# cybera/distributed_tensorflow_ibm_mnist

Measured on AMD Instinct MI355X. Metric: images/sec (whole node) MNIST LeNet-5, higher is better.
Workload: dtype bf16; 1 GPU; model=LeNet-5, global_batch=65536, per_gpu_batch=65536, parallelism=dp1, impl=hip, hip_graph=False, optimizer=momentum, input=bf16, input_lookahead=True

## Files before the change

### csrc/kernels/lenet_bwd.hip

```cpp
#include <cstdlib>
#include <cstring>

#include "common.h"
#include "launchers.h"
#include "wgrad_tr.h"

namespace mnistx {
namespace {


constexpr int NT = 1024, NW = 16, T = 8;
constexpr int NWIN1 = 196;
constexpr int AF_OFF = 0, AF_SZ = 15 * 64 * 16;
constexpr int DY2_RS = 384, DY2_IMG = 3872;
constexpr int DY2_OFF = AF_OFF + AF_SZ, DY2_SZ = T * DY2_IMG;
constexpr int ZERO_OFF = DY2_OFF + DY2_SZ;
constexpr int P1_RS = 272, P1_IMG = 3808;
constexpr int P1_OFF = ZERO_OFF + DY2_RS, P1_SZ = T * P1_IMG;
constexpr int X_RS = 80, X_IMG = 2592;
constexpr int X_OFF = P1_OFF + P1_SZ, X_SZ = T * X_IMG;
constexpr int D_RS = 280, D_IMG = 3920;
constexpr int DP1_OFF = X_OFF + X_SZ, D_SZ = T * D_IMG;
constexpr int CD_OFF = DP1_OFF + D_SZ;
constexpr int LDS_BYTES = CD_OFF + D_SZ;
static_assert(LDS_BYTES <= 163840, "one workgroup per CU");
static_assert(10 * DY2_RS <= DY2_IMG && 32 * X_RS <= X_IMG && 14 * P1_RS <= P1_IMG && 14 * D_RS <= D_IMG, "");
static_assert((ZERO_OFF - DY2_OFF) % 256 == 0, "zero row bank-aligned with the dY2 rows (bench/lds_bwd.py)");
constexpr int C2MAX = 4;
static_assert(NW * C2MAX * 256 * 4 <= LDS_BYTES && NW * 6 * 256 * 4 + NW * 8 * 4 <= LDS_BYTES, "epilogue scratch");

constexpr int C2_TAP0[13] = {0, 2, 5, 7, 10, 12, 15, 17, 20, 22, 4, 14, 24};
constexpr int C2_GT[4][C2MAX] = {{0, 1, 2, 3}, {4, 5, 10, -1}, {6, 7, 11, -1}, {8, 9, 12, -1}};
__constant__ int c2_gt[4][C2MAX] = {{0, 1, 2, 3}, {4, 5, 10, -1}, {6, 7, 11, -1}, {8, 9, 12, -1}};
__constant__ int c2_tap0[13] = {0, 2, 5, 7, 10, 12, 15, 17, 20, 22, 4, 14, 24};

struct BwdArgs {
  const bf16_t* x;
  const uint8_t* u8;
  const int64_t* idx;
  int n;
  const bf16_t* p1;
  const bf16_t* dp2;
  const uint8_t* arg2;
  const bf16_t* w2;
  int B;
  float* slab1;
  float* slab2;
  unsigned long long* prof;
  int skip;
  int prof_waves;
  int8_t du[16], k20[16], k21[16], k10[8], k11[8];
};
constexpr int NPROF = 8;

constexpr int NCH = 2;
static_assert(NW == 2 * T && 2 * 128 >= NWIN1 && 128 <= NWIN1, "staging: one wave pair per image, 2 chunks");
template <bool U8, bool IDX>
struct Stage {
  u32x2 x[NCH];
  u32x2 rowv;
  u32x4 dp;
  u32x2 c2;
  u32x4 p1[NCH];

  DEV static int img_of(int wave) { return wave >> 1; }
  DEV void load_row(const BwdArgs& a, int t0, int wave) {
    if constexpr (IDX) {
      const int img = img_of(wave);
      const bool ok = t0 >= 0 && t0 + img < a.B;
      const auto ridx = buf_rsrc(a.idx + (ok ? t0 + img : 0), ok ? 8u : 0u);
      rowv = buf_b64(ridx, 0u);
    }
  }
  DEV void load_xc(const BwdArgs& a, int t0, int wave, int ln) {
    const int img = img_of(wave);
    const bool ok = t0 >= 0 && t0 + img < a.B;
    int row = ok ? t0 + img : 0;
    if constexpr (IDX) {
      const uint32_t lo = __builtin_amdgcn_readfirstlane(rowv[0]), hi = __builtin_amdgcn_readfirstlane(rowv[1]);
      row = (hi != 0u || (int)lo < 0) ? 0 : ((int)lo >= a.n ? a.n - 1 : (int)lo);
    }
    constexpr uint32_t esz = U8 ? 1u : 2u;
    const void* xb = U8 ? (const void*)(a.u8 + (int64_t)row * 784) : (const void*)(a.x + (int64_t)row * 784);
    const auto rx = buf_rsrc(xb, ok ? 784u * esz : 0u);
    const int r = ln + 64 * (wave & 1);
#pragma unroll
    for (int i = 0; i < NCH; ++i) {
      const uint32_t q = (uint32_t)(r + 128 * i);
      const uint32_t oob = q < NWIN1 ? 0u : BUF_OOB;
      if constexpr (U8) x[i] = u32x2{buf_b32(rx, 4u * q + oob), 0u};
      else x[i] = buf_b64(rx, 8u * q + oob);
    }
  }
  DEV void store_xc(uint8_t* lds, int wave, int ln) const {
    const int img = img_of(wave), r = ln + 64 * (wave & 1);
#pragma unroll
    for (int i = 0; i < NCH; ++i) {
      const int q = r + 128 * i;
      if (i == 0 || q < NWIN1) {
        const int y = (q * 147) >> 10, k = q - 7 * y;
        const int yp = (q * 147) >> 11, xp = q - 14 * yp;
        uint32_t lo = x[i][0], hi = x[i][1];
        if constexpr (U8) {
          const uint32_t b = x[i][0];
          lo = pack2(u8_norm(b & 0xff), u8_norm((b >> 8) & 0xff));
          hi = pack2(u8_norm((b >> 16) & 0xff), u8_norm(b >> 24));
        }
        *(u32x2*)(lds + X_OFF + img * X_IMG + (y + 2) * X_RS + (4 * k + 4) * 2) = u32x2{lo, hi};
        const uint32_t a1 = p1[i][3];
        const uint32_t l4 = a1 & 0x0f0f0f0fu, h4 = (a1 >> 4) & 0x0f0f0f0fu;
        uint8_t* cd = lds + CD_OFF + img * D_IMG + yp * D_RS + xp * 16;
        *(u32x2*)cd = u32x2{bytes01(l4), bytes23(l4)};
        *(u32x2*)(cd + 8) = u32x2{bytes01(h4), bytes23(h4)};
      }
    }
  }
  DEV void load_dy(const BwdArgs& a, int t0, int wave, int ln) {
    const int nimg = t0 < 0 ? 0 : min(T, a.B - t0);
    const int tb = t0 < 0 ? 0 : t0;
    const int tid = wave * 64 + ln;
    const auto rdp = buf_rsrc(a.dp2 + (int64_t)tb * 400, (uint32_t)nimg * 800u);
    const auto ra2 = buf_rsrc(a.arg2 + (int64_t)tb * 400, (uint32_t)nimg * 400u);
    dp = buf_b128(rdp, tid < 400 ? 16u * tid : BUF_OOB);
    c2 = buf_b64(ra2, tid < 400 ? 8u * tid : BUF_OOB);
    const int img = img_of(wave);
    const bool ok = t0 >= 0 && t0 + img < a.B;
    const auto rp1 = buf_rsrc(a.p1 + (int64_t)(ok ? t0 + img : 0) * NWIN1 * 8, ok ? NWIN1 * 16u : 0u);
    const int r = ln + 64 * (wave & 1);
#pragma unroll
    for (int i = 0; i < NCH; ++i) {
      const uint32_t q = (uint32_t)(r + 128 * i);
      p1[i] = a.skip & 32 ? u32x4{0u, 0u, 0u, 0u} : buf_b128(rp1, q < NWIN1 ? 16u * q : BUF_OOB);
    }
  }
  DEV void store_dy(uint8_t* lds, int wave, int ln) {
    asm volatile("" : "+v"(dp), "+v"(c2), "+v"(p1[0]), "+v"(p1[1]));
    const int img = img_of(wave), r = ln + 64 * (wave & 1);
#pragma unroll
    for (int i = 0; i < NCH; ++i) {
      const int q = r + 128 * i;
      if (i == 0 || q < NWIN1) {
        const int yp = (q * 147) >> 11, xp = q - 14 * yp;
        const u32x4 v = {p1[i][0], p1[i][1], p1[i][2], 0x3f80u};
        *(u32x4*)(lds + P1_OFF + img * P1_IMG + yp * P1_RS + xp * 16) = v;
      }
    }
    const int tid = wave * 64 + ln;
    if (tid < 400) {
      const int im = tid / 50, rr = tid - 50 * im, w = rr >> 1, yp = w / 5, xp = w - 5 * yp;
      const int o = DY2_OFF + im * DY2_IMG + 2 * yp * DY2_RS + 2 * xp * 32 + 16 * (rr & 1);
      const uint32_t e[4] = {bytes01(c2[0]), bytes23(c2[0]), bytes01(c2[1]), bytes23(c2[1])};
      const int rot = (xp >> 1) & 1;
#pragma unroll
      for (int i = 0; i < 4; ++i) {
        const int d = i ^ rot;
        const uint32_t dd = (uint32_t)d * 0x00010001u;
        const u32x4 v = {sel_eq(dp[0], e[0], dd), sel_eq(dp[1], e[1], dd), sel_eq(dp[2], e[2], dd),
                         sel_eq(dp[3], e[3], dd)};
        *(u32x4*)(lds + o + (i >> 1) * DY2_RS + (d & 1) * 32) = v;
      }
    }
  }
};

template <int H>
DEV void dgrad_unit(const uint8_t* lds, int bB, int bZ, int orow, int lane, int dylo, int dyhi, f32x4 (&acc)[4]) {
  constexpr int VLO = H ? 2 : 0, VHI = H ? 4 : 3, NU = H ? 3 : 4;
#pragma unroll 2
  for (int dy = dylo; dy <= dyhi; ++dy) {
    bf16x8 Bv[VHI - VLO + 1];
    const int r = orow - dy;
    const uint8_t* pb = lds + ((unsigned)r <= 9u ? bB - dy * DY2_RS : bZ);
#pragma unroll
    for (int v = VLO; v <= VHI; ++v) Bv[v - VLO] = *(const bf16x8*)(pb + 64 * v);
#pragma unroll
    for (int j = 0; j < 3; ++j) {
      const bf16x8 A = *(const bf16x8*)(lds + AF_OFF + ((dy * 3 + j) * 64 + lane) * 16);
#pragma unroll
      for (int v = VLO; v <= VHI; ++v) {
        const int u = v + 2 - j - 4 * H;
        if (u >= 0 && u < NU) acc[u] = mfma16(A, Bv[v - VLO], acc[u]);
      }
    }
  }
}

template <int G>
DEV void c2w_steps(const uint8_t* lds, int ks0, int ks1, int ln, f32x4 (&acc2)[C2MAX]) {
  const int g = ln >> 4, q = (ln >> 2) & 3, p = ln & 3;
  const int img = 4 * (g & 1) + q, sub = 2 * (g >> 1), hA = p >> 1, pc = p & 1;
  const int bB = DY2_OFF + img * DY2_IMG + sub * 32 + 8 * p;
  const int aB = P1_OFF + img * P1_IMG + sub * 16 + 8 * pc;
  const int aP = aB + hA * 16, aR = aB + hA * P1_RS;
  constexpr int NT2 = G == 0 ? 4 : 3;
#pragma unroll 2
  for (int s = ks0; s < ks1; ++s) {
    const int y = s / 3, x0 = 4 * (s - 3 * y);
    const int sb = bB + y * DY2_RS + x0 * 32, sa = y * P1_RS + x0 * 16;
    const bf16x8 Bf = frag(tr4(lds, sb), tr4(lds, sb + 32));
#pragma unroll
    for (int t = 0; t < NT2; ++t) {
      const int tile = C2_GT[G][t], tap = C2_TAP0[tile];
      const int base = (tile < 10 ? aP : aR) + sa + (tap / 5) * P1_RS + (tap % 5) * 16;
      acc2[t] = mfma16(frag(tr4(lds, base), tr4(lds, base + 16)), Bf, acc2[t]);
    }
  }
}

constexpr int8_t DG_UNIT[NW] = {7, 5, 9, 4, 6, 10, 3, 8, 2, 11, 0, 1, 12, 13, -1, -1};
constexpr int8_t C2_KS0[NW] = {0, 6, 13, 23, 0, 8, 16, 23, 0, 7, 15, 22, 0, 7, 14, 22};
constexpr int8_t C2_KS1[NW] = {6, 13, 23, 30, 8, 16, 23, 30, 7, 15, 22, 30, 7, 14, 22, 30};
constexpr int8_t C1_KS0[8] = {0, 4, 8, 12, 16, 20, 24, 26};
constexpr int8_t C1_KS1[8] = {4, 8, 12, 16, 20, 24, 26, 28};

template <bool PROF, bool U8, bool IDX>
__global__ __launch_bounds__(NT, 1) void lenet_bwd_k(const BwdArgs a) {
  extern __shared__ __attribute__((aligned(16))) uint8_t lds[];
  const int tid = threadIdx.x, lane = tid & 63, wave = __builtin_amdgcn_readfirstlane(tid >> 6);
  const int ntiles = (a.B + T - 1) / T;
  const int nk = ntiles > (int)blockIdx.x ? (ntiles - 1 - (int)blockIdx.x) / (int)gridDim.x + 1 : 0;
  auto tile0 = [&](int k) { return k < nk ? ((int)blockIdx.x + k * (int)gridDim.x) * T : -1; };

  for (int e = tid; e < LDS_BYTES / 16; e += NT) *(u32x4*)(lds + 16 * e) = u32x4{0u, 0u, 0u, 0u};
  __syncthreads();
  if (tid < 15 * 64) {
    const int f = tid >> 6, dy = f / 3, j = f - 3 * dy;
    const int r = (lane & 15) >> 3, ci = lane & 7, xs = lane >> 5, co0 = 8 * ((lane >> 4) & 1);
    const int dx = r + 4 - 2 * j - xs;
    u32x4 v = {0u, 0u, 0u, 0u};
    if (dx >= 0 && dx <= 4) v = *(const u32x4*)(a.w2 + ((dy * 5 + dx) * 8 + ci) * 16 + co0);
    *(u32x4*)(lds + AF_OFF + 16 * tid) = v;
  }
  Stage<U8, IDX> st;
  st.load_row(a, tile0(0), wave);
  st.load_xc(a, tile0(0), wave, lane);
  st.load_dy(a, tile0(0), wave, lane);
  st.load_row(a, tile0(1), wave);
  st.store_dy(lds, wave, lane);

  const int grp = wave >> 2, sig = wave & 1;
  f32x4 acc2[C2MAX];
#pragma unroll
  for (int t = 0; t < C2MAX; ++t) acc2[t] = f32x4{0.f, 0.f, 0.f, 0.f};
  f32x4 acc1[3][2];
#pragma unroll
  for (int t = 0; t < 3; ++t) acc1[t][0] = acc1[t][1] = f32x4{0.f, 0.f, 0.f, 0.f};
  float db1[4] = {0.f, 0.f, 0.f, 0.f};
  const int du = a.du[wave];
  const int ks0 = a.k20[wave], ks1 = a.k21[wave];
  const int cs0 = a.k10[wave >> 1], cs1 = a.k11[wave >> 1];

  uint64_t pc_acc[NPROF] = {0, 0, 0, 0, 0, 0, 0, 0};
  uint64_t tclk = __builtin_amdgcn_s_memtime();
  auto mark = [&](int ph) {
    if constexpr (PROF) {
      const uint64_t t = __builtin_amdgcn_s_memtime();
      pc_acc[ph] += t - tclk;
      tclk = t;
    }
  };

  for (int k = 0; k < nk; ++k) {
    const int t0 = tile0(k);
    if (!(PROF && (a.skip & 16))) __syncthreads();
    mark(6);
    if (!(PROF && (a.skip & 8))) {
      const int ln = lane_now();
      st.store_xc(lds, wave, ln);
    }
    mark(0);

    if (du >= 0 && !(PROF && (a.skip & 1))) {
      const int ln = lane_now();
      const int i16 = ln & 15, g = ln >> 4;
      const int pr = du >> 1, hx = du & 1;
      const int img = i16 >> 1, rr = i16 & 1, orow = 2 * pr + rr;
      const int dylo = max(0, 2 * pr - 9), dyhi = min(4, 2 * pr + 1);
      const int u0 = 4 * hx;
      u32x2 pv[4];
#pragma unroll
      for (int u = 0; u < 4; ++u)
        pv[u] = *(const u32x2*)(lds + P1_OFF + img * P1_IMG + orow * P1_RS + (2 * min(u0 + u, 6) + (g >> 1)) * 16 +
                                8 * (g & 1));
      if (!(PROF && (a.skip & 8))) st.load_xc(a, tile0(k + 1), wave, ln);
      f32x4 acc[4];
#pragma unroll
      for (int u = 0; u < 4; ++u) acc[u] = f32x4{0.f, 0.f, 0.f, 0.f};
      const int lo = (g >> 1) * 32 + (g & 1) * 16;
      const int bB = DY2_OFF + img * DY2_IMG + orow * DY2_RS + lo, bZ = ZERO_OFF + lo;
      if (hx) dgrad_unit<1>(lds, bB, bZ, orow, ln, dylo, dyhi, acc);
      else dgrad_unit<0>(lds, bB, bZ, orow, ln, dylo, dyhi, acc);
      const int wB = DP1_OFF + img * D_IMG + orow * D_RS + (2 * u0 + (g >> 1)) * 16 + 8 * (g & 1);
#pragma unroll
      for (int u = 0; u < 4; ++u) {
        if (u0 + u < 7) {
          *(u32x2*)(lds + wB + 32 * u) = u32x2{pack2(acc[u][0], acc[u][1]), pack2(acc[u][2], acc[u][3])};
#pragma unroll
          for (int i = 0; i < 4; ++i) {
            const int16_t pvi = (int16_t)((pv[u][i >> 1] >> (16 * (i & 1))) & 0xffffu);
            db1[i] = fmaf(acc[u][i], pvi > 0 ? 1.f : 0.f, db1[i]);
          }
        }
      }
    } else if (!(PROF && (a.skip & 8))) {
      st.load_xc(a, tile0(k + 1), wave, lane_now());
    }
    if (!(PROF && (a.skip & 8))) st.load_dy(a, tile0(k + 1), wave, lane_now());
    mark(1);

    if (ks0 < ks1 && !(PROF && (a.skip & 2))) {
      const int ln = lane_now();
      switch (grp) {
        case 0: c2w_steps<0>(lds, ks0, ks1, ln, acc2); break;
        case 1: c2w_steps<1>(lds, ks0, ks1, ln, acc2); break;
        case 2: c2w_steps<2>(lds, ks0, ks1, ln, acc2); break;
        default: c2w_steps<3>(lds, ks0, ks1, ln, acc2); break;
      }
    }

    mark(2);
    if (!(PROF && (a.skip & 16))) __syncthreads();
    mark(3);
    if (!(PROF && (a.skip & 8))) st.load_row(a, tile0(k + 2), wave);
    mark(4);

    {
      const int ln = lane_now(), g = ln >> 4, q = (ln >> 2) & 3, p = ln & 3;
      const int img = 4 * (g & 1) + q, sub = 2 * (g >> 1), hA = p >> 1, pc = p & 1;
      const uint32_t dsel = (uint32_t)((ln & 15) >> 3);
      const uint32_t dd0 = dsel * 0x00010001u, dd1 = (2u + dsel) * 0x00010001u;
      const int aB = X_OFF + img * X_IMG + hA * X_RS + (4 * sub + 4 * pc + 4 * sig) * 2;
      const int bB = DP1_OFF + img * D_IMG + (2 * sub + sig) * 16 + 8 * pc;
#pragma unroll 2
      for (int s = cs0; s < (PROF && (a.skip & 4) ? cs0 : cs1); ++s) {
        const int yp = s >> 1, xi0 = 4 * (s & 1);
        const int sa = aB + 2 * yp * X_RS + 8 * xi0, sb = bB + yp * D_RS + 32 * xi0;
        const u32x4 dv = __builtin_bit_cast(u32x4, frag(tr4(lds, sb), tr4(lds, sb + 32)));
        const u32x4 cv = __builtin_bit_cast(u32x4, frag(tr4(lds, sb + (CD_OFF - DP1_OFF)),
                                                         tr4(lds, sb + (CD_OFF - DP1_OFF) + 32)));
        const bf16x8 B0 = __builtin_bit_cast(bf16x8, u32x4{sel_eq(dv[0], cv[0], dd0), sel_eq(dv[1], cv[1], dd0),
                                                           sel_eq(dv[2], cv[2], dd0), sel_eq(dv[3], cv[3], dd0)});
        const bf16x8 B1 = __builtin_bit_cast(bf16x8, u32x4{sel_eq(dv[0], cv[0], dd1), sel_eq(dv[1], cv[1], dd1),
                                                           sel_eq(dv[2], cv[2], dd1), sel_eq(dv[3], cv[3], dd1)});
#pragma unroll
        for (int t = 0; t < 3; ++t) {
          const bf16x8 Af = frag(tr4(lds, sa + 2 * t * X_RS), tr4(lds, sa + 2 * t * X_RS + 8));
          acc1[t][0] = mfma16(Af, B0, acc1[t][0]);
          acc1[t][1] = mfma16(Af, B1, acc1[t][1]);
        }
      }
    }
    if (k + 1 < nk && !(PROF && (a.skip & 8))) st.store_dy(lds, wave, lane_now());
    mark(5);
  }

  const int i16 = lane & 15, g = lane >> 4;
  __syncthreads();
  mark(6);
  float* e2 = (float*)lds;
#pragma unroll
  for (int t = 0; t < C2MAX; ++t) *(f32x4*)(e2 + ((wave * C2MAX + t) * 16 + i16) * 16 + 4 * g) = acc2[t];
  __syncthreads();
  float* s2 = a.slab2 + (int64_t)blockIdx.x * 208 * 16;
  for (int e = tid; e < 4 * C2MAX * 256; e += NT) {
    const int G = e >> 10, t = (e >> 8) & 3, row = (e >> 4) & 15, col = e & 15;
    const int tile = c2_gt[G][t];
    if (tile < 0) continue;
    const int h = row >> 3, ci = row & 7, tap = c2_tap0[tile] + h * (tile < 10 ? 1 : 5);
    const bool bias = tile == 0 && h == 0 && ci == 6;
    if (tap >= 25 || (ci >= 6 && !bias)) continue;
    float v = 0.f;
#pragma unroll
    for (int w = 0; w < 4; ++w) v += e2[(((4 * G + w) * C2MAX + t) * 16 + col) * 16 + row];
    s2[(bias ? 200 : tap * 8 + ci) * 16 + col] = v;
  }
  __syncthreads();
  float* e1 = (float*)lds;
#pragma unroll
  for (int t = 0; t < 3; ++t)
#pragma unroll
    for (int nt = 0; nt < 2; ++nt)
      *(f32x4*)(e1 + (((wave * 3 + t) * 2 + nt) * 16 + i16) * 16 + 4 * g) = acc1[t][nt];
#pragma unroll
  for (int i = 0; i < 4; ++i) {
#pragma unroll
    for (int m = 1; m <= 32; m = m == 8 ? 32 : 2 * m) db1[i] += __shfl_xor(db1[i], m);
  }
  float* eb = e1 + NW * 6 * 256;
  if (lane == 0 || lane == 16) *(f32x4*)(eb + wave * 8 + (lane >> 2)) = f32x4{db1[0], db1[1], db1[2], db1[3]};
  __syncthreads();
  float* s1 = a.slab1 + (int64_t)blockIdx.x * 32 * 8;
  if (tid < 26 * 8) {
    const int tap = tid >> 3, c = tid & 7;
    float v = 0.f;
    if (tap < 25) {
      const int dy = tap / 5, dx = tap - 5 * dy;
      for (int w = 0; w < NW; ++w) {
        const int s = w & 1;
#pragma unroll
        for (int d = 0; d < 4; ++d) {
          const int ty = dy + (d >> 1), tx = dx + (d & 1), txi = tx + (s ? 0 : 2);
          const int t = ty >> 1, row = 4 * (2 * (ty & 1) + (txi >> 2)) + (txi & 3);
          const int nt = d >> 1, col = c + 8 * (d & 1);
          v += e1[(((w * 3 + t) * 2 + nt) * 16 + col) * 16 + row];
        }
      }
    } else {
      for (int w = 0; w < NW; ++w) v += eb[w * 8 + c];
    }
    s1[tap * 8 + c] = v;
  }
  if constexpr (PROF) {
    mark(7);
    __syncthreads();
    unsigned long long* ep = (unsigned long long*)lds;
    if (lane == 0)
      for (int i = 0; i < NPROF; ++i) ep[wave * NPROF + i] = pc_acc[i];
    __syncthreads();
    if (tid < NPROF) {
      unsigned long long v = 0;
      for (int w = 0; w < NW; ++w) v += ep[w * NPROF + tid];
      atomicAdd(a.prof + tid, v);
    }
    if (a.prof_waves && tid < NW * NPROF) atomicAdd(a.prof + NPROF + tid, ep[tid]);
  }
}

struct BwdSplit {
  int8_t du[16], k20[16], k21[16], k10[8], k11[8];
  bool ok;
};
BwdSplit bwd_split() {
  BwdSplit s{};
  memcpy(s.du, DG_UNIT, 16);
  memcpy(s.k20, C2_KS0, 16);
  memcpy(s.k21, C2_KS1, 16);
  memcpy(s.k10, C1_KS0, 8);
  memcpy(s.k11, C1_KS1, 8);
  s.ok = true;
  const char* e = getenv("MNISTX_BWD_SPLIT");
  if (!e || !*e) return s;
  int v[64], n = 0;
  for (const char* p = e; *p && n < 64;) {
    char* end = nullptr;
    const long x = strtol(p, &end, 10);
    if (end == p) break;
    v[n++] = (int)x;
    p = *end == ',' ? end + 1 : end;
  }
  if (n != 64) return BwdSplit{{}, {}, {}, {}, {}, false};
  int seen[14] = {};
  for (int w = 0; w < 16; ++w) {
    if (v[w] < -1 || v[w] > 13) return BwdSplit{{}, {}, {}, {}, {}, false};
    if (v[w] >= 0) ++seen[v[w]];
  }
  for (int u = 0; u < 14; ++u)
    if (seen[u] != 1) return BwdSplit{{}, {}, {}, {}, {}, false};
  for (int G = 0; G < 4; ++G) {
    int cover[30] = {};
    for (int t = 0; t < 4; ++t) {
      const int w = 4 * G + t, k0 = v[16 + w], k1 = v[32 + w];
      if (k0 < 0 || k1 < k0 || k1 > 30) return BwdSplit{{}, {}, {}, {}, {}, false};
      for (int k = k0; k < k1; ++k) ++cover[k];
    }
    for (int k = 0; k < 30; ++k)
      if (cover[k] != 1) return BwdSplit{{}, {}, {}, {}, {}, false};
  }
  int cover1[28] = {};
  for (int r = 0; r < 8; ++r) {
    const int k0 = v[48 + r], k1 = v[56 + r];
    if (k0 < 0 || k1 < k0 || k1 > 28) return BwdSplit{{}, {}, {}, {}, {}, false};
    for (int k = k0; k < k1; ++k) ++cover1[k];
  }
  for (int k = 0; k < 28; ++k)
    if (cover1[k] != 1) return BwdSplit{{}, {}, {}, {}, {}, false};
  for (int i = 0; i < 16; ++i) {
    s.du[i] = (int8_t)v[i];
    s.k20[i] = (int8_t)v[16 + i];
    s.k21[i] = (int8_t)v[32 + i];
  }
  for (int i = 0; i < 8; ++i) {
    s.k10[i] = (int8_t)v[48 + i];
    s.k11[i] = (int8_t)v[56 + i];
  }
  return s;
}

using BwdKernel = void (*)(BwdArgs);
constexpr BwdKernel kBwd[8] = {lenet_bwd_k<false, false, false>, lenet_bwd_k<false, false, true>,
                               lenet_bwd_k<false, true, false>,  lenet_bwd_k<false, true, true>,
                               lenet_bwd_k<true, false, false>,  lenet_bwd_k<true, false, true>,
                               lenet_bwd_k<true, true, false>,   lenet_bwd_k<true, true, true>};

}

int lenet_bwd_grid(int* per_cu = nullptr) {
  static int n = 0, per = 0;
  if (n == 0) {
    int dev = 0, cus = 0;
    for (BwdKernel k : kBwd)
      if (hipFuncSetAttribute((const void*)k, hipFuncAttributeMaxDynamicSharedMemorySize, LDS_BYTES) != hipSuccess)
        return -1;
    if (hipOccupancyMaxActiveBlocksPerMultiprocessor(&per, kBwd[0], NT, LDS_BYTES) != hipSuccess ||
        hipGetDevice(&dev) != hipSuccess ||
        hipDeviceGetAttribute(&cus, hipDeviceAttributeMultiprocessorCount, dev) != hipSuccess || per <= 0)
      return -1;
    n = per * cus;
  }
  if (per_cu) *per_cu = per;
  return n;
}

hipError_t lenet_bwd(const XSrc& x, const bf16_t* p1, const bf16_t* dp2, const uint8_t* arg2, const bf16_t* w2,
                     int B, float* slab1, float* slab2, int grid, hipStream_t st, unsigned long long* prof) {
  if (B <= 0) return hipSuccess;
  if ((!x.x && !x.u8) || grid <= 0) return hipErrorInvalidValue;
  const int res = lenet_bwd_grid();
  if (res <= 0) return hipErrorInvalidValue;
  BwdArgs a{x.u8 ? nullptr : x.x, x.u8, x.idx, x.idx ? x.n : B, p1, dp2, arg2, w2, B, slab1, slab2, prof, 0, 0,
            {}, {}, {}, {}, {}};
  static const BwdSplit sp = bwd_split();
  if (!sp.ok) return hipErrorInvalidValue;
  memcpy(a.du, sp.du, 16);
  memcpy(a.k20, sp.k20, 16);
  memcpy(a.k21, sp.k21, 16);
  memcpy(a.k10, sp.k10, 8);
  memcpy(a.k11, sp.k11, 8);
  if (prof) {
    const char* e = getenv("MNISTX_BWD_SKIP");
    a.skip = e ? atoi(e) : 0;
    const char* pw = getenv("MNISTX_BWD_PROF_WAVES");
    a.prof_waves = (pw && pw[0] == '1') ? 1 : 0;
  }
  const BwdKernel k = kBwd[(prof ? 4 : 0) + (x.u8 ? 2 : 0) + (x.idx ? 1 : 0)];
  void* args[] = {&a};
  return hipLaunchKernel((const void*)k, dim3(grid), dim3(NT), args, LDS_BYTES, st);
}

int lenet_bwd_blocks(int B) {
  int per = 1;
  const int full = lenet_bwd_grid(&per);
  if (full <= 0) return -1;
  const int res = reserve_cut(full, per);
  const int ntiles = (B + T - 1) / T;
  return cap_grid(ntiles < res ? ntiles : res);
}

}
```

Baseline: 168.8 million images/s.

## Software-pipeline LDS loads against MFMAs in backward dgrad and wgrad loops

Adds pipelined versions of the conv2 dgrad, conv2 wgrad and conv1 wgrad inner loops. Each loop prefetches the next step's A/B fragments from LDS while the current step's MFMAs issue, and uses sched_barrier to keep that interleaving fixed. The goal is to hide LDS latency behind matrix-core work, at the cost of more live registers and a fixed instruction schedule. The pipelined kernel is the default and can be turned off with the MNISTX_BWD_PIPE=0 environment variable.

```diff
diff --git a/csrc/kernels/lenet_bwd.hip b/csrc/kernels/lenet_bwd.hip
--- a/csrc/kernels/lenet_bwd.hip
+++ b/csrc/kernels/lenet_bwd.hip
@@ -9,6 +9,9 @@
 namespace {
 
 
+#ifndef BWD_PIPE_LOOPS
+#define BWD_PIPE_LOOPS 7
+#endif
 constexpr int NT = 1024, NW = 16, T = 8;
 constexpr int NWIN1 = 196;
 constexpr int AF_OFF = 0, AF_SZ = 15 * 64 * 16;
@@ -115,6 +118,11 @@
       }
     }
   }
+  DEV void drop_xc() { x[0] = x[1] = u32x2{0u, 0u}; }
+  DEV void drop_dy() {
+    dp = p1[0] = p1[1] = u32x4{0u, 0u, 0u, 0u};
+    c2 = u32x2{0u, 0u};
+  }
   DEV void load_dy(const BwdArgs& a, int t0, int wave, int ln) {
     const int nimg = t0 < 0 ? 0 : min(T, a.B - t0);
     const int tb = t0 < 0 ? 0 : t0;
@@ -182,6 +190,53 @@
         if (u >= 0 && u < NU) acc[u] = mfma16(A, Bv[v - VLO], acc[u]);
       }
     }
+  }
+}
+
+constexpr int8_t DG_J[2][9] = {{0, 1, 2, 0, 1, 2, 1, 2, 2}, {0, 0, 0, 1, 1, 2, -1, -1, -1}};
+constexpr int8_t DG_V[2][9] = {{0, 0, 0, 1, 1, 1, 2, 2, 3}, {2, 3, 4, 3, 4, 4, -1, -1, -1}};
+constexpr bool dg_last_j(int H, int n) {
+  for (int m = n + 1; m < 9; ++m)
+    if (DG_J[H][m] == DG_J[H][n]) return false;
+  return true;
+}
+constexpr bool dg_last_v(int H, int n) {
+  for (int m = n + 1; m < 9; ++m)
+    if (DG_V[H][m] == DG_V[H][n]) return false;
+  return true;
+}
+template <int H>
+DEV void dgrad_unit_pipe(const uint8_t* lds, int bB, int bZ, int orow, int lane, int dylo, int dyhi,
+                         f32x4 (&acc)[4]) {
+  constexpr int VLO = H ? 2 : 0, VHI = H ? 4 : 3, NM = H ? 6 : 9;
+  auto rowp = [&](int dy) {
+    const int r = orow - dy;
+    return lds + ((unsigned)r <= 9u ? bB - dy * DY2_RS : bZ);
+  };
+  auto ldA = [&](int dy, int j) { return *(const bf16x8*)(lds + AF_OFF + ((dy * 3 + j) * 64 + lane) * 16); };
+  bf16x8 Bv[VHI - VLO + 1], A[3];
+  {
+    const uint8_t* pb = rowp(dylo);
+#pragma unroll
+    for (int v = VLO; v <= VHI; ++v) Bv[v - VLO] = *(const bf16x8*)(pb + 64 * v);
+#pragma unroll
+    for (int j = 0; j < 3; ++j) A[j] = ldA(dylo, j);
+  }
+  for (int dy = dylo; dy < dyhi; ++dy) {
+    const uint8_t* pn = rowp(dy + 1);
+#pragma unroll
+    for (int n = 0; n < NM; ++n) {
+      const int j = DG_J[H][n], v = DG_V[H][n], u = v + 2 - j - 4 * H;
+      acc[u] = mfma16(A[j], Bv[v - VLO], acc[u]);
+      __builtin_amdgcn_sched_barrier(0);
+      if (dg_last_j(H, n)) A[j] = ldA(dy + 1, j);
+      if (dg_last_v(H, n)) Bv[v - VLO] = *(const bf16x8*)(pn + 64 * v);
+    }
+  }
+#pragma unroll
+  for (int n = 0; n < NM; ++n) {
+    const int j = DG_J[H][n], v = DG_V[H][n], u = v + 2 - j - 4 * H;
+    acc[u] = mfma16(A[j], Bv[v - VLO], acc[u]);
   }
 }
 
@@ -207,13 +262,124 @@
   }
 }
 
+template <int G>
+DEV void c2w_steps_pipe(const uint8_t* lds, int ks0, int ks1, int ln, f32x4 (&acc2)[C2MAX]) {
+  if (ks0 >= ks1) return;
+  const int g = ln >> 4, q = (ln >> 2) & 3, p = ln & 3;
+  const int img = 4 * (g & 1) + q, sub = 2 * (g >> 1), hA = p >> 1, pc = p & 1;
+  const int bB = DY2_OFF + img * DY2_IMG + sub * 32 + 8 * p;
+  const int aB = P1_OFF + img * P1_IMG + sub * 16 + 8 * pc;
+  const int aP = aB + hA * 16, aR = aB + hA * P1_RS;
+  constexpr int NT2 = G == 0 ? 4 : 3;
+  auto ldB = [&](int s) {
+    const int y = s / 3, x0 = 4 * (s - 3 * y);
+    const int sb = bB + y * DY2_RS + x0 * 32;
+    return frag(tr4(lds, sb), tr4(lds, sb + 32));
+  };
+  auto ldA = [&](int s, int t) {
+    const int y = s / 3, x0 = 4 * (s - 3 * y);
+    const int tile = C2_GT[G][t], tap = C2_TAP0[tile];
+    const int base = (tile < 10 ? aP : aR) + y * P1_RS + x0 * 16 + (tap / 5) * P1_RS + (tap % 5) * 16;
+    return frag(tr4(lds, base), tr4(lds, base + 16));
+  };
+  bf16x8 A[NT2], Ba = ldB(ks0), Bb;
+#pragma unroll
+  for (int t = 0; t < NT2; ++t) A[t] = ldA(ks0, t);
+  auto step = [&](int sn, const bf16x8& Bc, bf16x8& Bn) {
+    Bn = ldB(sn);
+#pragma unroll
+    for (int t = 0; t < NT2; ++t) {
+      acc2[t] = mfma16(A[t], Bc, acc2[t]);
+      __builtin_amdgcn_sched_barrier(0);
+      A[t] = ldA(sn, t);
+    }
+  };
+  auto drain = [&](const bf16x8& Bc) {
+#pragma unroll
+    for (int t = 0; t < NT2; ++t) acc2[t] = mfma16(A[t], Bc, acc2[t]);
+  };
+  int sn = ks0 + 1;
+  for (; sn + 1 < ks1; sn += 2) {
+    step(sn, Ba, Bb);
+    step(sn + 1, Bb, Ba);
+  }
+  if (sn < ks1) {
+    step(sn, Ba, Bb);
+    drain(Bb);
+  } else {
+    drain(Ba);
+  }
+}
+
+DEV void c1w_steps_pipe(const uint8_t* lds, int cs0, int cs1, int ln, int sig, f32x4 (&acc1)[3][2]) {
+  if (cs0 >= cs1) return;
+  const int g = ln >> 4, q = (ln >> 2) & 3, p = ln & 3;
+  const int img = 4 * (g & 1) + q, sub = 2 * (g >> 1), hA = p >> 1, pc = p & 1;
+  const uint32_t dsel = (uint32_t)((ln & 15) >> 3);
+  const uint32_t dd0 = dsel * 0x00010001u, dd1 = (2u + dsel) * 0x00010001u;
+  const int aB = X_OFF + img * X_IMG + hA * X_RS + (4 * sub + 4 * pc + 4 * sig) * 2;
+  const int bB = DP1_OFF + img * D_IMG + (2 * sub + sig) * 16 + 8 * pc;
+  auto ldA = [&](int s, int t) {
+    const int sa = aB + 2 * (s >> 1) * X_RS + 32 * (s & 1) + 2 * t * X_RS;
+    return frag(tr4(lds, sa), tr4(lds, sa + 8));
+  };
+  auto ldD = [&](int s, u32x4& dv, u32x4& cv) {
+    const int sb = bB + (s >> 1) * D_RS + 128 * (s & 1);
+    dv = __builtin_bit_cast(u32x4, frag(tr4(lds, sb), tr4(lds, sb + 32)));
+    cv = __builtin_bit_cast(u32x4, frag(tr4(lds, sb + (CD_OFF - DP1_OFF)), tr4(lds, sb + (CD_OFF - DP1_OFF) + 32)));
+  };
+  auto mask = [&](const u32x4& dv, const u32x4& cv, uint32_t dd) {
+    return __builtin_bit_cast(bf16x8, u32x4{sel_eq(dv[0], cv[0], dd), sel_eq(dv[1], cv[1], dd),
+                                            sel_eq(dv[2], cv[2], dd), sel_eq(dv[3], cv[3], dd)});
+  };
+  bf16x8 A[3], Ba[2], Bb[2];
+  {
+    u32x4 dv, cv;
+    ldD(cs0, dv, cv);
+#pragma unroll
+    for (int t = 0; t < 3; ++t) A[t] = ldA(cs0, t);
+    Ba[0] = mask(dv, cv, dd0);
+    Ba[1] = mask(dv, cv, dd1);
+  }
+  auto step = [&](int sn, const bf16x8 (&Bc)[2], bf16x8 (&Bn)[2]) {
+    u32x4 dv, cv;
+    ldD(sn, dv, cv);
+#pragma unroll
+    for (int t = 0; t < 3; ++t) {
+      acc1[t][0] = mfma16(A[t], Bc[0], acc1[t][0]);
+      acc1[t][1] = mfma16(A[t], Bc[1], acc1[t][1]);
+      __builtin_amdgcn_sched_barrier(0);
+      A[t] = ldA(sn, t);
+      if (t > 0) Bn[t - 1] = mask(dv, cv, t == 1 ? dd0 : dd1);
+    }
+  };
+  auto drain = [&](const bf16x8 (&Bc)[2]) {
+#pragma unroll
+    for (int t = 0; t < 3; ++t) {
+      acc1[t][0] = mfma16(A[t], Bc[0], acc1[t][0]);
+      acc1[t][1] = mfma16(A[t], Bc[1], acc1[t][1]);
+    }
+  };
+  int sn = cs0 + 1;
+  for (; sn + 1 < cs1; sn += 2) {
+    step(sn, Ba, Bb);
+    step(sn + 1, Bb, Ba);
+  }
+  if (sn < cs1) {
+    step(sn, Ba, Bb);
+    drain(Bb);
+  } else {
+    drain(Ba);
+  }
+}
+
 constexpr int8_t DG_UNIT[NW] = {7, 5, 9, 4, 6, 10, 3, 8, 2, 11, 0, 1, 12, 13, -1, -1};
 constexpr int8_t C2_KS0[NW] = {0, 6, 13, 23, 0, 8, 16, 23, 0, 7, 15, 22, 0, 7, 14, 22};
 constexpr int8_t C2_KS1[NW] = {6, 13, 23, 30, 8, 16, 23, 30, 7, 15, 22, 30, 7, 14, 22, 30};
 constexpr int8_t C1_KS0[8] = {0, 4, 8, 12, 16, 20, 24, 26};
 constexpr int8_t C1_KS1[8] = {4, 8, 12, 16, 20, 24, 26, 28};
 
-template <bool PROF, bool U8, bool IDX>
+template <bool PIPE, bool PROF, bool U8, bool IDX>
 __global__ __launch_bounds__(NT, 1) void lenet_bwd_k(const BwdArgs a) {
   extern __shared__ __attribute__((aligned(16))) uint8_t lds[];
   const int tid = threadIdx.x, lane = tid & 63, wave = __builtin_amdgcn_readfirstlane(tid >> 6);
@@ -277,19 +443,30 @@
       const int img = i16 >> 1, rr = i16 & 1, orow = 2 * pr + rr;
       const int dylo = max(0, 2 * pr - 9), dyhi = min(4, 2 * pr + 1);
       const int u0 = 4 * hx;
+      constexpr bool DPIPE = PIPE && (BWD_PIPE_LOOPS & 1);
       u32x2 pv[4];
-#pragma unroll
-      for (int u = 0; u < 4; ++u)
-        pv[u] = *(const u32x2*)(lds + P1_OFF + img * P1_IMG + orow * P1_RS + (2 * min(u0 + u, 6) + (g >> 1)) * 16 +
-                                8 * (g & 1));
+      auto load_pv = [&] {
+#pragma unroll
+        for (int u = 0; u < 4; ++u)
+          pv[u] = *(const u32x2*)(lds + P1_OFF + img * P1_IMG + orow * P1_RS + (2 * min(u0 + u, 6) + (g >> 1)) * 16 +
+                                  8 * (g & 1));
+      };
+      if constexpr (!DPIPE) load_pv();
       if (!(PROF && (a.skip & 8))) st.load_xc(a, tile0(k + 1), wave, ln);
+      else st.drop_xc();
       f32x4 acc[4];
 #pragma unroll
       for (int u = 0; u < 4; ++u) acc[u] = f32x4{0.f, 0.f, 0.f, 0.f};
       const int lo = (g >> 1) * 32 + (g & 1) * 16;
       const int bB = DY2_OFF + img * DY2_IMG + orow * DY2_RS + lo, bZ = ZERO_OFF + lo;
-      if (hx) dgrad_unit<1>(lds, bB, bZ, orow, ln, dylo, dyhi, acc);
-      else dgrad_unit<0>(lds, bB, bZ, orow, ln, dylo, dyhi, acc);
+      if constexpr (DPIPE) {
+        if (hx) dgrad_unit_pipe<1>(lds, bB, bZ, orow, ln, dylo, dyhi, acc);
+        else dgrad_unit_pipe<0>(lds, bB, bZ, orow, ln, dylo, dyhi, acc);
+        load_pv();
+      } else {
+        if (hx) dgrad_unit<1>(lds, bB, bZ, orow, ln, dylo, dyhi, acc);
+        else dgrad_unit<0>(lds, bB, bZ, orow, ln, dylo, dyhi, acc);
+      }
       const int wB = DP1_OFF + img * D_IMG + orow * D_RS + (2 * u0 + (g >> 1)) * 16 + 8 * (g & 1);
 #pragma unroll
       for (int u = 0; u < 4; ++u) {
@@ -304,17 +481,29 @@
       }
     } else if (!(PROF && (a.skip & 8))) {
       st.load_xc(a, tile0(k + 1), wave, lane_now());
+    } else {
+      st.drop_xc();
     }
     if (!(PROF && (a.skip & 8))) st.load_dy(a, tile0(k + 1), wave, lane_now());
+    else st.drop_dy();
     mark(1);
 
     if (ks0 < ks1 && !(PROF && (a.skip & 2))) {
       const int ln = lane_now();
-      switch (grp) {
-        case 0: c2w_steps<0>(lds, ks0, ks1, ln, acc2); break;
-        case 1: c2w_steps<1>(lds, ks0, ks1, ln, acc2); break;
-        case 2: c2w_steps<2>(lds, ks0, ks1, ln, acc2); break;
-        default: c2w_steps<3>(lds, ks0, ks1, ln, acc2); break;
+      if constexpr (PIPE && (BWD_PIPE_LOOPS & 2)) {
+        switch (grp) {
+          case 0: c2w_steps_pipe<0>(lds, ks0, ks1, ln, acc2); break;
+          case 1: c2w_steps_pipe<1>(lds, ks0, ks1, ln, acc2); break;
+          case 2: c2w_steps_pipe<2>(lds, ks0, ks1, ln, acc2); break;
+          default: c2w_steps_pipe<3>(lds, ks0, ks1, ln, acc2); break;
+        }
+      } else {
+        switch (grp) {
+          case 0: c2w_steps<0>(lds, ks0, ks1, ln, acc2); break;
+          case 1: c2w_steps<1>(lds, ks0, ks1, ln, acc2); break;
+          case 2: c2w_steps<2>(lds, ks0, ks1, ln, acc2); break;
+          default: c2w_steps<3>(lds, ks0, ks1, ln, acc2); break;
+        }
       }
     }
 
@@ -324,7 +513,9 @@
     if (!(PROF && (a.skip & 8))) st.load_row(a, tile0(k + 2), wave);
     mark(4);
 
-    {
+    if constexpr (PIPE && (BWD_PIPE_LOOPS & 4)) {
+      c1w_steps_pipe(lds, cs0, PROF && (a.skip & 4) ? cs0 : cs1, lane_now(), sig, acc1);
+    } else {
       const int ln = lane_now(), g = ln >> 4, q = (ln >> 2) & 3, p = ln & 3;
       const int img = 4 * (g & 1) + q, sub = 2 * (g >> 1), hA = p >> 1, pc = p & 1;
       const uint32_t dsel = (uint32_t)((ln & 15) >> 3);
@@ -487,10 +678,13 @@
 }
 
 using BwdKernel = void (*)(BwdArgs);
-constexpr BwdKernel kBwd[8] = {lenet_bwd_k<false, false, false>, lenet_bwd_k<false, false, true>,
-                               lenet_bwd_k<false, true, false>,  lenet_bwd_k<false, true, true>,
-                               lenet_bwd_k<true, false, false>,  lenet_bwd_k<true, false, true>,
-                               lenet_bwd_k<true, true, false>,   lenet_bwd_k<true, true, true>};
+#define BWD_K8(PIPE)                                                                                   \
+  lenet_bwd_k<PIPE, false, false, false>, lenet_bwd_k<PIPE, false, false, true>,                       \
+      lenet_bwd_k<PIPE, false, true, false>, lenet_bwd_k<PIPE, false, true, true>,                     \
+      lenet_bwd_k<PIPE, true, false, false>, lenet_bwd_k<PIPE, true, false, true>,                     \
+      lenet_bwd_k<PIPE, true, true, false>, lenet_bwd_k<PIPE, true, true, true>
+constexpr BwdKernel kBwd[16] = {BWD_K8(false), BWD_K8(true)};
+#undef BWD_K8
 
 }
 
@@ -532,7 +726,9 @@
     const char* pw = getenv("MNISTX_BWD_PROF_WAVES");
     a.prof_waves = (pw && pw[0] == '1') ? 1 : 0;
   }
-  const BwdKernel k = kBwd[(prof ? 4 : 0) + (x.u8 ? 2 : 0) + (x.idx ? 1 : 0)];
+  const char* pe = getenv("MNISTX_BWD_PIPE");
+  const bool pipe = !(pe && pe[0] == '0');
+  const BwdKernel k = kBwd[(pipe ? 8 : 0) + (prof ? 4 : 0) + (x.u8 ? 2 : 0) + (x.idx ? 1 : 0)];
   void* args[] = {&a};
   return hipLaunchKernel((const void*)k, dim3(grid), dim3(NT), args, LDS_BYTES, st);
 }
```

Result: faster. 172.1 million images/s (median of 6 runs) (+2.0%).
